# renmengye/rec-attend-public

Hardware: AMD Instinct MI355X
Metric: instance-timesteps/sec, full_model forward 512x512 T=16 (whole job; pipelined throughput: 8 batches in flight per GPU, fill and drain of the pipeline inside the timed region; config.lone_batch_* = one sync-bracketed forward) (higher is better)
Workload: dtype f32; 1 GPU; cfg2: CVPPP-arch full_model eval forward, 512x512, T=16, B=8 per GPU, y_out+s_out; arch=cvppp, H=512, W=512, T=16, batch_per_gpu=8, global_batch=8, parallelism=batch-sharded x1, no collective, ranks_in_communicator=1, hip_graph=True, tile_tickets=False, batches_in_flight=8, pipeline_slots=4, batches_per_launch=2, input=resident in HBM, output=left in HBM

## Files before the change

rec-attend-public_amd/csrc/ra_conv_pair8.hip:

```cpp
#include "ra_conv_pair_parts.h"
#include "ra_split3.h"

namespace ra {
namespace cpair {

template <int CINA>
struct NGeo {
  static constexpr int TH = 16, TW = 32;
  static constexpr int NCGA = CINA / 4;
  static constexpr int AGX = 5, AGY = 5, NGA = AGX * AGY, GPW = (NGA + 3) / 4;
  static constexpr int AW = 41, AHS = TH + 2;
  static constexpr int LW = 43, LH = 4 * AGY + 2;
  static constexpr int LHL = TH + 4, LWL = TW + 6;
  static constexpr int PLANE_B = AHS * AW * 16;
  template <bool CACHED>
  static constexpr int tin_floats() {
    return (LH * LW * (CACHED ? 1 : CINA) + 3) & ~3;
  }
  template <bool SPLIT>
  static constexpr int tmid_floats() {
    return SPLIT ? 3 * PLANE_B / 4 : AHS * AW * 8;
  }
  template <bool CACHED, bool SPLIT>
  static constexpr int lds_floats() {
    return tin_floats<CACHED>() + tmid_floats<SPLIT>();
  }
};

#ifndef RA_PAIR8_OCC
#define RA_PAIR8_OCC 3
#endif
#ifdef RA_PROBE8
__device__ long long *ra_probe8_buf;
#define RA_PHASE_PROBE_BUF ra_probe8_buf
#define RA_PHASE_PROBE_WG blockIdx.x
#endif
#include "ra_phase_probe.h"
#ifdef RA_P8_NOBAR
#define RA_P8_SYNC() __builtin_amdgcn_s_waitcnt(0xc07f)
#else
#define RA_P8_SYNC() __syncthreads()
#endif
template <int CINA, bool CACHED, bool SPLIT = false>
__global__ __launch_bounds__(256, CACHED ? (SPLIT ? 3 : 4) : RA_PAIR8_OCC) void conv_pair8_mfma(const PArgs a, int tiles_x, int tiles_y, int ntiles) {
  using G = NGeo<CINA>;
  constexpr int NCGA = G::NCGA;
  static_assert(!CACHED || CINA == 4, "cached form: 4 input channels");
  static_assert(!SPLIT || CACHED, "the split-precision layer B exists for the cached (steady-state) form");
  constexpr int PLANE_B = G::PLANE_B;
  constexpr int RECA = CACHED ? 1 : CINA;
  extern __shared__ __attribute__((aligned(16))) float lds[];
  constexpr int IN_FLOATS = G::template tin_floats<CACHED>();
  float *tin = lds;
  float *tmid = lds + IN_FLOATS;
  typedef typename vec_of<NCGA>::type avecA;

  const int tid = threadIdx.x, lane = tid & 63;
  __shared__ unsigned tk_sh[2];
  TicketWalk tk;
  const bool dyn = a.tickets != nullptr;
  if (dyn) tk.issue(a.tickets, ntiles);
  const int wave = __builtin_amdgcn_readfirstlane(tid >> 6);
  const int m = lane & 15, ksub = lane >> 4;
  const int n = lane & 15, qo = lane >> 4;
  const int p = n >> 3, co = n & 7;
  const int per = tiles_x * tiles_y;

  const float scA = a.scA[co], scB = a.scB[co], shB = a.shB[co];
  const float loA = a.reluA ? 0.f : -__builtin_inff(), loB = a.reluB ? 0.f : -__builtin_inff();
  const int qA = m >> 2, rA = m & 3, pA = ksub >> 1, coA0 = 4 * (ksub & 1);
  f32x4 scA4, shA4;
#pragma unroll
  for (int j = 0; j < 4; ++j) scA4[j] = a.scA[coA0 + j], shA4[j] = a.shA[coA0 + j];
  const bool fill = !CACHED && a.cache != nullptr;
  float bA[CACHED ? 1 : 12][NCGA], bB[12][2];
  float bAc[3];
#pragma unroll
  for (int ky = 0; ky < 3; ++ky) {
    const int kx = ksub - p;
    const bool ok = (kx >= 0) & (kx <= 2);
    const int tap = ok ? ky * 3 + kx : 0;
    const float w = a.wpA[((tap * NCGA + (a.plane_chan >> 2)) * 4 + (a.plane_chan & 3)) * a.CoutAP + co];
    bAc[ky] = (CACHED && ok) ? w * scA : 0.f;
  }
#pragma unroll
  for (int ky = 0; ky < 3; ++ky)
#pragma unroll
    for (int kxp = 0; kxp < 4; ++kxp) {
      const int kx = kxp - p;
      const bool ok = (kx >= 0) & (kx <= 2);
      const int tap = ok ? ky * 3 + kx : 0;
      if constexpr (!CACHED) {
#pragma unroll
        for (int cg = 0; cg < NCGA; ++cg) {
          const float w = a.wpA[((tap * NCGA + cg) * 4 + ksub) * a.CoutAP + co];
          bA[ky * 4 + kxp][cg] = ok ? w * (fill ? 1.f : scA) : 0.f;
        }
      }
#pragma unroll
      for (int cg = 0; cg < 2; ++cg) {
        const float w = a.wpB[((tap * 2 + cg) * 4 + ksub) * a.CoutBP + co];
        bB[ky * 4 + kxp][cg] = ok ? w * scB : 0.f;
      }
    }

  s16x8 wB[SPLIT ? 3 : 1][SPLIT ? 3 : 1];
  if constexpr (SPLIT) {
#pragma unroll
    for (int ky = 0; ky < 3; ++ky) {
      const int kx = ksub - p;
      const bool ok = (kx >= 0) & (kx <= 2);
      const int tap = ok ? ky * 3 + kx : 0;
#pragma unroll
      for (int j = 0; j < 8; j += 2) {
        const float w0 = a.wpB[((tap * 2 + (j >> 2)) * 4 + (j & 3)) * a.CoutBP + co];
        const float w1 = a.wpB[((tap * 2 + ((j + 1) >> 2)) * 4 + ((j + 1) & 3)) * a.CoutBP + co];
        unsigned H, M, L;
        split3_pair(ok ? w0 * scB : 0.f, ok ? w1 * scB : 0.f, H, M, L);
        wB[ky][0][j] = (short)(H & 0xffffu), wB[ky][0][j + 1] = (short)(H >> 16);
        wB[ky][1][j] = (short)(M & 0xffffu), wB[ky][1][j + 1] = (short)(M >> 16);
        wB[ky][2][j] = (short)(L & 0xffffu), wB[ky][2][j + 1] = (short)(L >> 16);
      }
    }
  }
  const __amdgpu_buffer_rsrc_t rs = __builtin_amdgcn_make_buffer_rsrc(const_cast<float *>(a.src), 0, a.bytes0, 0x00020000);
  const __amdgpu_buffer_rsrc_t rp = __builtin_amdgcn_make_buffer_rsrc(
      const_cast<float *>(a.plane ? a.plane : a.src), 0, a.plane ? a.bytes_p : 0, 0x00020000);
  constexpr int NE = G::LHL * G::LWL, NIT = (NE + 255) / 256;
  int e_rr[NIT], e_cc[NIT];
#pragma unroll
  for (int i = 0; i < NIT; ++i) {
    const int e = tid + 256 * i;
    e_rr[i] = e / G::LWL;
    e_cc[i] = e - e_rr[i] * G::LWL;
    if (e >= NE) e_rr[i] = -(1 << 20);
  }
  unsigned e_offp[NIT], e_offs[NIT];
#pragma unroll
  for (int i = 0; i < NIT; ++i) {
    const bool in = tid + 256 * i < NE;
    const unsigned o = (unsigned)(e_rr[i] * a.W + e_cc[i]) * 4u;
    e_offp[i] = in ? o : 0x80000000u;
    e_offs[i] = in ? o * CINA : 0x80000000u;
  }
  struct TC {
    int b, ty, tx;
  };
  auto split = [&](int t) {
    TC c;
    c.b = t / per;
    const int r = t - c.b * per;
    c.ty = r / tiles_x;
    c.tx = r - c.ty * tiles_x;
    return c;
  };
  const int nwx = a.xcd_map ? (int)gridDim.x >> 3 : (int)gridDim.x;
  const int chunk = (ntiles + 7) >> 3;
  const int t_first = a.xcd_map ? ((int)blockIdx.x & 7) * chunk + ((int)blockIdx.x >> 3) : (int)blockIdx.x;
  const int t_end = a.xcd_map ? (((int)blockIdx.x & 7) * chunk + chunk < ntiles ? ((int)blockIdx.x & 7) * chunk + chunk : ntiles) : ntiles;
  const TC stride = split(nwx);
  auto advance = [&](TC c) {
    c.tx += stride.tx;
    if (c.tx >= tiles_x) {
      c.tx -= tiles_x;
      ++c.ty;
    }
    c.ty += stride.ty;
    if (c.ty >= tiles_y) {
      c.ty -= tiles_y;
      ++c.b;
    }
    c.b += stride.b;
    return c;
  };
  f32x4 v[NIT][NCGA];
  float pv[NIT];
  auto fetch = [&](const TC &c) {
    const int fb = c.b, fy0 = c.ty * G::TH - 2, fx0 = c.tx * G::TW - 3;
    const bool inside = (fy0 >= 0) & (fy0 + G::LHL <= a.H) & (fx0 >= 0) & (fx0 + G::LWL <= a.W);
    if (inside) {
      const unsigned base = (unsigned)((fb * a.H + fy0) * a.W + fx0) * 4u;
#pragma unroll
      for (int i = 0; i < NIT; ++i) {
        if constexpr (!CACHED) {
#pragma unroll
          for (int cg = 0; cg < NCGA; ++cg)
            v[i][cg] = __builtin_bit_cast(
                f32x4, __builtin_amdgcn_raw_buffer_load_b128(rs, (int)(base * CINA + e_offs[i] + 16u * cg), 0, 0));
        }
        pv[i] = __builtin_bit_cast(float, __builtin_amdgcn_raw_buffer_load_b32(rp, (int)(base + e_offp[i]), 0, 0));
      }
      return;
    }
#pragma unroll
    for (int i = 0; i < NIT; ++i) {
      const int Y = fy0 + e_rr[i], X = fx0 + e_cc[i];
      const bool ok = (Y >= 0) & (Y < a.H) & (X >= 0) & (X < a.W);
      const int pix = (fb * a.H + Y) * a.W + X;
      if constexpr (!CACHED) {
#pragma unroll
        for (int cg = 0; cg < NCGA; ++cg)
          v[i][cg] = __builtin_bit_cast(
              f32x4, __builtin_amdgcn_raw_buffer_load_b128(rs, ok ? (pix * CINA + 4 * cg) * 4 : 0x7fffffff, 0, 0));
      }
      pv[i] = __builtin_bit_cast(float, __builtin_amdgcn_raw_buffer_load_b32(rp, ok ? pix * 4 : 0x7fffffff, 0, 0));
    }
  };

  const int lane_in = CACHED ? (m >> 2) * G::LW + 2 * (m & 3) + ksub
                             : ((m >> 2) * G::LW + 2 * (m & 3)) * CINA + ksub * NCGA;
  const __amdgpu_buffer_rsrc_t rc = __builtin_amdgcn_make_buffer_rsrc(
      const_cast<float *>(a.cache ? a.cache : a.src), 0, a.cache ? a.bytes_c : 0, 0x00020000);
  const int lane_b = ((m & 1) * G::AW + 2 * (m >> 1) + 1) * 8 + ksub * 2;
  const int pg = a.plane_chan >> 2, slot = a.plane_chan & 3;

  int slot_c[G::GPW];
#pragma unroll
  for (int s = 0; s < G::GPW; ++s) {
    int gi = wave + 4 * s;
    if (gi >= G::NGA) gi = G::NGA - 1;
    const int gr = gi / G::AGX, gc = gi - gr * G::AGX;
    slot_c[s] = (4 * gr * a.cache_gx + gc) * 256;
  }
  const int lane_c = qA * a.cache_gx * 256 + rA * 64 + ksub * 16;
  const __amdgpu_buffer_rsrc_t ry = __builtin_amdgcn_make_buffer_rsrc(a.y, 0, a.bytes_y, 0x00020000);
  const unsigned lane_y = co < a.CoutB ? (unsigned)(((2 * qo + p) * a.CoutB + co) * 4) : 0x80000000u;
  int g_y[4];
#pragma unroll
  for (int g = 0; g < 4; ++g) g_y[g] = ((g >> 1) * a.Wo + 8 * (g & 1)) * a.CoutB * 4;

  int tile = t_first;
  if (dyn) {
    tk.begin(tk_sh);
    tile = tk.cur;
  }
  bool have = dyn ? tile >= 0 : tile < t_end;
  TC cur = split(have ? tile : 0), nxt = cur;
  if (have) fetch(cur);
  RA_PHASE_DECL;
  for (int e = tid; e < G::template lds_floats<CACHED, SPLIT>() / 4; e += 256)
    reinterpret_cast<f32x4 *>(lds)[e] = f32x4{0.f, 0.f, 0.f, 0.f};
  __syncthreads();
  const bool rider = !CACHED && a.rider_dst != nullptr;
  const __amdgpu_buffer_rsrc_t rr = __builtin_amdgcn_make_buffer_rsrc(rider ? a.rider_dst : a.y, 0,
                                                                       rider ? a.rider_quads * 16 : 0, 0x00020000);
  const int r_chunk = rider ? (a.rider_quads + (int)gridDim.x - 1) / (int)gridDim.x : 0;
  int r_idx = (int)blockIdx.x * r_chunk + tid;
  const int r_end = ((int)blockIdx.x + 1) * r_chunk < a.rider_quads ? ((int)blockIdx.x + 1) * r_chunk : a.rider_quads;
  const int my_tiles = t_end > t_first ? (t_end - t_first + nwx - 1) / nwx : 1;
  const int r_per_tile = (r_chunk + 256 * my_tiles - 1) / (256 * my_tiles);
  const u32x4 r_bits = __builtin_bit_cast(u32x4, f32x4{a.rider_val, a.rider_val, a.rider_val, a.rider_val});
  bool have_n = false;
  f32x4 cpre[CACHED ? G::GPW : 1];
  auto load_cache = [&](const TC &tc) {
    const int tile_c0 = ((tc.b * a.cache_rows + tc.ty * G::TH) * a.cache_gx + ((tc.tx * G::TW) >> 3)) * 256;
#pragma unroll
    for (int s = 0; s < (CACHED ? G::GPW : 1); ++s)
      cpre[s] = __builtin_bit_cast(f32x4, __builtin_amdgcn_raw_buffer_load_b128(rc, tile_c0 + slot_c[s] + lane_c, 0, 0));
  };
  for (; have; tile = dyn ? (tk.step(), tk.cur) : tile + nwx, cur = nxt, have = have_n) {
    const int b = cur.b, ty0 = cur.ty * G::TH, tx0 = cur.tx * G::TW;
    if constexpr (CACHED) load_cache(cur);

#pragma unroll
    for (int i = 0; i < NIT; ++i) {
      if constexpr (CACHED) {
        if (e_rr[i] >= 0) tin[e_rr[i] * G::LW + e_cc[i]] = pv[i];
        continue;
      }
      if (a.plane) {
#pragma unroll
        for (int cg = 0; cg < NCGA; ++cg) {
          v[i][cg].x = (cg == pg && slot == 0) ? pv[i] : v[i][cg].x;
          v[i][cg].y = (cg == pg && slot == 1) ? pv[i] : v[i][cg].y;
          v[i][cg].z = (cg == pg && slot == 2) ? pv[i] : v[i][cg].z;
          v[i][cg].w = (cg == pg && slot == 3) ? pv[i] : v[i][cg].w;
        }
      }
      if (e_rr[i] >= 0) {
        float *rec = tin + (e_rr[i] * G::LW + e_cc[i]) * CINA;
        if constexpr (NCGA == 1) {
          *reinterpret_cast<f32x4 *>(rec) = v[i][0];
        } else {
#pragma unroll
          for (int ks = 0; ks < 4; ++ks)
#pragma unroll
            for (int cg = 0; cg < NCGA; ++cg) rec[ks * NCGA + cg] = v[i][cg][ks];
        }
      }
    }
    if (dyn) tk.publish(tk_sh);
    RA_P8_SYNC();
    RA_PHASE_AT(0);
    if (dyn) {
      tk.read_next(tk_sh);
      tk.request();
      have_n = tk.nxt >= 0;
      nxt = split(have_n ? tk.nxt : 0);
    } else {
      have_n = tile + nwx < t_end;
      nxt = advance(cur);
    }
    if (have_n) fetch(nxt);
    if constexpr (!CACHED) {
      if (rider)
        for (int u = 0; u < r_per_tile; ++u, r_idx += 256)
          __builtin_amdgcn_raw_buffer_store_b128(r_bits, rr, r_idx < r_end ? r_idx * 16 : 0x7fffffff, 0, 0);
    }

    {
      const bool interior = (ty0 >= 1) & (ty0 + G::TH + 1 <= a.H) & (tx0 >= 2) & (tx0 + G::TW + 1 <= a.W);
      const int tile_c = ((b * a.cache_rows + ty0) * a.cache_gx + (tx0 >> 3)) * 256;
      f32x4 acc[G::GPW];
      int gin[G::GPW];
#pragma unroll
      for (int s = 0; s < G::GPW; ++s) {
        int gi = wave + 4 * s;
        if (gi >= G::NGA) gi = G::NGA - 1;
        const int gr = gi / G::AGX, gc = gi - gr * G::AGX;
        gin[s] = (4 * gr * G::LW + 8 * gc) * RECA + lane_in;
        if constexpr (CACHED) {
          acc[s] = cpre[s] * scA4 + shA4;
        } else {
          acc[s] = fill ? f32x4{0.f, 0.f, 0.f, 0.f} : shA4;
        }
      }
      RA_PHASE_AT(1);
      if constexpr (CACHED) {
#pragma unroll
        for (int ky = 0; ky < 3; ++ky) {
          float av[G::GPW];
#pragma unroll
          for (int s = 0; s < G::GPW; ++s) av[s] = tin[gin[s] + ky * G::LW];
#pragma unroll
          for (int s = 0; s < G::GPW; ++s)
            acc[s] = __builtin_amdgcn_mfma_f32_16x16x4f32(bAc[ky], av[s], acc[s], 0, 0, 0);
        }
      } else {
#pragma unroll
      for (int ky = 0; ky < 3; ++ky)
#pragma unroll
        for (int kxp = 0; kxp < 4; ++kxp) {
          avecA av[G::GPW];
#pragma unroll
          for (int s = 0; s < G::GPW; ++s)
            av[s] = *reinterpret_cast<const avecA *>(&tin[gin[s] + (ky * G::LW + kxp) * CINA]);
#pragma unroll
          for (int cg = 0; cg < NCGA; ++cg)
#pragma unroll
            for (int s = 0; s < G::GPW; ++s)
              acc[s] = __builtin_amdgcn_mfma_f32_16x16x4f32(bA[ky * 4 + kxp][cg], av[s][cg], acc[s], 0, 0, 0);
        }
      }
      if (fill) {
#pragma unroll
        for (int s = 0; s < G::GPW; ++s) {
          int gi = wave + 4 * s;
          if (gi >= G::NGA) gi = G::NGA - 1;
          const int gr = gi / G::AGX, gc = gi - gr * G::AGX;
          const bool mine = (4 * gr + qA < G::AHS) & ((gc < 4) | (tx0 + G::TW >= a.W));
          const int off = mine ? tile_c + slot_c[s] + lane_c : 0x7fffffff;
          __builtin_amdgcn_raw_buffer_store_b128(__builtin_bit_cast(__attribute__((ext_vector_type(4))) unsigned, acc[s]), rc, off, 0, 0);
          acc[s] = acc[s] * scA4 + shA4;
        }
      }
#pragma unroll
      for (int s = 0; s < G::GPW; ++s) {
        const int gi = wave + 4 * s;
        const int gr = gi / G::AGX, gc = gi - gr * G::AGX;
        const bool live = (gi < G::NGA) & (4 * gr + qA < G::AHS);
        float o[4];
#pragma unroll
        for (int j = 0; j < 4; ++j) o[j] = fmaxf(acc[s][j], loA);
        if (!interior) {
          const int Y = ty0 - 1 + 4 * gr + qA, X = tx0 - 2 + 8 * gc + 2 * rA + pA;
          const bool ok = (Y >= 0) & (Y < a.H) & (X >= 0) & (X < a.W);
#pragma unroll
          for (int j = 0; j < 4; ++j) o[j] = ok ? o[j] : 0.f;
        }
        const int pix = (4 * gr + qA) * G::AW + 8 * gc + 2 * rA + pA;
        if constexpr (SPLIT) {
          unsigned H01, M01, L01, H23, M23, L23;
          split3_pair(o[0], o[1], H01, M01, L01);
          split3_pair(o[2], o[3], H23, M23, L23);
          if (live) {
            unsigned char *d0 = reinterpret_cast<unsigned char *>(tmid) + pix * 16 + coA0 * 2;
            *reinterpret_cast<u32x2 *>(d0) = u32x2{H01, H23};
            *reinterpret_cast<u32x2 *>(d0 + PLANE_B) = u32x2{M01, M23};
            *reinterpret_cast<u32x2 *>(d0 + 2 * PLANE_B) = u32x2{L01, L23};
          }
        } else if (live) {
          float *dst = tmid + pix * 8 + (ksub & 1);
#pragma unroll
          for (int j = 0; j < 4; ++j) dst[2 * j] = o[j];
        }
      }
    }
    RA_PHASE_AT(2);
    RA_P8_SYNC();
    RA_PHASE_AT(3);

    {
      f32x4 acc[4];
      int gmid[4];
#pragma unroll
      for (int g = 0; g < 4; ++g) {
        const int gy = 2 * wave + (g >> 1), gx = g & 1;
        gmid[g] = (2 * gy * G::AW + 16 * gx) * 8 + lane_b;
        acc[g] = f32x4{shB, shB, shB, shB};
      }
      if constexpr (SPLIT) {
        const unsigned char *tb = reinterpret_cast<const unsigned char *>(tmid);
        const int lane_px = ((m & 1) * G::AW + 2 * (m >> 1) + 1 + ksub) * 16;
#pragma unroll
        for (int ky = 0; ky < 3; ++ky)
#pragma unroll
          for (int gh = 0; gh < 2; ++gh) {
            s16x8 av[2][3];
#pragma unroll
            for (int u = 0; u < 2; ++u) {
              const int g = 2 * gh + u;
              const int gy = 2 * wave + (g >> 1), gx = g & 1;
              const int off = ((2 * gy + ky) * G::AW + 16 * gx) * 16 + lane_px;
#pragma unroll
              for (int pc = 0; pc < 3; ++pc) av[u][pc] = *reinterpret_cast<const s16x8 *>(tb + off + pc * PLANE_B);
            }
            constexpr int PA[6] = {1, 0, 2, 0, 1, 0}, PB[6] = {1, 2, 0, 1, 0, 0};
#pragma unroll
            for (int t = 0; t < 6; ++t)
#pragma unroll
              for (int u = 0; u < 2; ++u)
                acc[2 * gh + u] = __builtin_amdgcn_mfma_f32_16x16x32_bf16(__builtin_bit_cast(bf16x8, av[u][PA[t]]),
                                                                          __builtin_bit_cast(bf16x8, wB[ky][PB[t]]), acc[2 * gh + u], 0, 0, 0);
          }
      } else {
#pragma unroll
      for (int ky = 0; ky < 3; ++ky)
#pragma unroll
        for (int kxp = 0; kxp < 4; ++kxp) {
          f32x2 av[4];
#pragma unroll
          for (int g = 0; g < 4; ++g)
            av[g] = *reinterpret_cast<const f32x2 *>(&tmid[gmid[g] + (ky * G::AW + kxp) * 8]);
#pragma unroll
          for (int cg = 0; cg < 2; ++cg)
#pragma unroll
            for (int g = 0; g < 4; ++g)
              acc[g] = __builtin_amdgcn_mfma_f32_16x16x4f32(av[g][cg], bB[ky * 4 + kxp][cg], acc[g], 0, 0, 0);
        }
      }
      const int prow0 = (ty0 >> 1) + wave * 2, pcol0 = (tx0 >> 1) + 2 * qo + p;
      const bool whole = ((ty0 >> 1) + G::TH / 2 <= a.Ho) & ((tx0 >> 1) + G::TW / 2 <= a.Wo);
      const unsigned tile_y = (unsigned)(((b * a.Ho + prow0) * a.Wo + (tx0 >> 1)) * a.CoutB * 4) + lane_y;
#pragma unroll
      for (int g = 0; g < 4; ++g) {
        const float t0 = fmaxf(fmaxf(acc[g][0], acc[g][1]), loB), t1 = fmaxf(fmaxf(acc[g][2], acc[g][3]), loB);
        const float u0 = fmaxf(t0, __builtin_bit_cast(float, __builtin_amdgcn_mov_dpp(__builtin_bit_cast(int, t0), 0x128, 0xf, 0xf, true)));
        const float u1 = fmaxf(t1, __builtin_bit_cast(float, __builtin_amdgcn_mov_dpp(__builtin_bit_cast(int, t1), 0x128, 0xf, 0xf, true)));
        const float ov = p ? u1 : u0;
        const int prow = prow0 + (g >> 1), pcol = pcol0 + 8 * (g & 1);
        unsigned off = tile_y + (unsigned)g_y[g];
        if (!whole) off = ((prow < a.Ho) & (pcol < a.Wo)) ? off : 0x80000000u;
        __builtin_amdgcn_raw_buffer_store_b32(__builtin_bit_cast(unsigned, ov), ry, (int)off, 0, 0);
      }
    }
    RA_PHASE_AT(4);
  }
  RA_PHASE_END;
  if constexpr (!CACHED) {
    if (rider)
      for (; r_idx < r_end; r_idx += 256) __builtin_amdgcn_raw_buffer_store_b128(r_bits, rr, r_idx * 16, 0, 0);
  }
}

template <int CINA, bool CACHED = false, bool SPLIT = false>
int launch8(PArgs a, int B, hipStream_t st, int *plan) {
  using G = NGeo<CINA>;
  a.bytes_y = (int)((size_t)B * a.Ho * a.Wo * a.CoutB * sizeof(float));
  auto kern = conv_pair8_mfma<CINA, CACHED, SPLIT>;
  constexpr size_t lds = (size_t)G::template lds_floats<CACHED, SPLIT>() * sizeof(float);
  const int tiles_x = ceil_div(a.W, G::TW), tiles_y = ceil_div(a.H, G::TH);
  const int ntiles = tiles_x * tiles_y * B;
  static const int wgs = env_int("RA_PAIR8_WGS", 768);
  static const int xcd = env_int("RA_PAIR8_XCD", 1);
  const int grid = ntiles < wgs ? ntiles : wgs;
  a.xcd_map = (xcd && grid % 8 == 0 && grid >= 8) ? 1 : 0;
  const bool draws = CACHED && ntiles >= kTicketMinTilesPerWg * grid;
  if (plan) {
    plan[RA_PLAN_FAMILY] = RA_PLAN_FAMILY_PAIR;
    plan[RA_PLAN_FORM] = RA_PLAN_FORM_NPACKED | (CACHED ? RA_PLAN_FORM_CACHED : 0) | (SPLIT ? RA_PLAN_FORM_SPLIT : 0);
    plan[RA_PLAN_CK] = CINA, plan[RA_PLAN_CMID] = 8, plan[RA_PLAN_KF] = 3, plan[RA_PLAN_TILE_H] = G::TH, plan[RA_PLAN_TILE_W] = G::TW;
    plan[RA_PLAN_TILES_X] = tiles_x, plan[RA_PLAN_TILES_Y] = tiles_y, plan[RA_PLAN_TICKETS] = draws ? 1 : 0;
    plan_walk(plan, ntiles, grid, a.xcd_map);
    return 0;
  }
  static const MaxDynamicLds lds_limit(kern, lds);
  a.tickets = draws ? take_ticket_slots(1, grid) : nullptr;
  hipLaunchKernelGGL(kern, dim3(grid), dim3(256), lds, st, a, tiles_x, tiles_y, ntiles);
  return launch_status("ra_conv_pair_f32");
}

__global__ __launch_bounds__(256) void first_cache_kernel(const float *x, const float *wpA, int CoutAP, int plane_chan,
                                                          int B, int H, int W, int rows, int ngx, float *cache) {
  __shared__ float sm[4][64][9];
  const int xl = threadIdx.x & 63, yl = threadIdx.x >> 6;
  const int X = blockIdx.x * 64 - 2 + xl, Y = blockIdx.y * 4 + yl, b = blockIdx.z;
  float acc[8];
#pragma unroll
  for (int co = 0; co < 8; ++co) acc[co] = 0.f;
  if (X >= 0 && X < W && Y < H) {
#pragma unroll
    for (int ky = 0; ky < 3; ++ky) {
      const int yy = Y + ky - 1;
#pragma unroll
      for (int kx = 0; kx < 3; ++kx) {
        const int xx = X + kx - 1;
        const bool ok = (yy >= 0) & (yy < H) & (xx >= 0) & (xx < W);
        f32x4 v = f32x4{0.f, 0.f, 0.f, 0.f};
        if (ok) v = *reinterpret_cast<const f32x4 *>(x + ((size_t)(b * H + yy) * W + xx) * 4);
        const float *wt = wpA + (size_t)((ky * 3 + kx) * 4) * CoutAP;
#pragma unroll
        for (int ci = 0; ci < 4; ++ci) {
          const float xv = ci == plane_chan ? 0.f : v[ci];
#pragma unroll
          for (int co = 0; co < 8; ++co) acc[co] = fmaf(xv, wt[ci * CoutAP + co], acc[co]);
        }
      }
    }
  }
#pragma unroll
  for (int co = 0; co < 8; ++co) sm[yl][xl][co] = acc[co];
  __syncthreads();
  for (int e = threadIdx.x; e < 4 * 8 * 16; e += 256) {
    const int n4 = e & 3, r = (e >> 2) & 3, g = (e >> 4) & 7, row = e >> 7;
    const int p = n4 >> 1, co0 = 4 * (n4 & 1);
    const int Yo = blockIdx.y * 4 + row, gx = blockIdx.x * 8 + g;
    if (Yo < H && gx < ngx) {
      f32x4 o;
#pragma unroll
      for (int j = 0; j < 4; ++j) o[j] = sm[row][8 * g + 2 * r + p][co0 + j];
      *reinterpret_cast<f32x4 *>(cache + (((size_t)b * rows + (Yo + 1)) * ngx + gx) * 64 + r * 16 + 4 * n4) = o;
    }
  }
}

void cache_dims(int H, int W, int &rows, int &ngx) {
  rows = ceil_div(H, NGeo<4>::TH) * NGeo<4>::TH + 4;
  ngx = ceil_div(W, NGeo<4>::TW) * (NGeo<4>::TW / 8) + 1;
}
int launch_npacked(const PArgs &a, int B, hipStream_t st, int *plan) {
  return a.C0 == 4 ? launch8<4>(a, B, st, plan) : launch8<8>(a, B, st, plan);
}

int fill_cache_entry(const float *src, const float *plane, int plane_chan, int B, int H, int W, const float *wpA, const float *scaleA,
                     const float *shiftA, int reluA, const float *wpB, const float *scaleB, const float *shiftB, int CoutB, int reluB,
                     float *cache, float *y, float *fill_dst, size_t fill_floats, float fill_value, void *stream, int *plan) {
  if (missing_pointer(plan, {src, plane, cache, wpA, scaleA, shiftA, wpB, scaleB, shiftB, y}) || B <= 0)
    return fail(RA_E_INVALID, "ra_conv_pair_fill_cache_f32: bad argument");
  if (fill_dst && ((reinterpret_cast<uintptr_t>(fill_dst) & 15) || (fill_floats & 3) || fill_floats * 4 >= (1ull << 31)))
    return fail(RA_E_SHAPE, "ra_conv_pair_fill_cache_rider_f32: the fill must be 16-byte aligned, a multiple of 4 floats, < 2 GiB");
  if (!ra_conv_first_cache_supported(4, 8, CoutB, 2, H, W) || plane_chan < 0 || plane_chan > 3)
    return fail(RA_E_SHAPE, "ra_conv_pair_fill_cache_f32: unsupported shape");
  PArgs a = pair_args(src, 4, B, H, W, 0, wpA, scaleA, shiftA, 8, reluA, wpB, scaleB, shiftB, CoutB, reluB, 2, plane, plane_chan, y);
  const size_t b0 = (size_t)B * H * W * 4 * sizeof(float);
  if (b0 >= (1ull << 31)) return fail(RA_E_SHAPE, "ra_conv_pair_fill_cache_f32: input exceeds 2 GiB");
  a.bytes0 = (int)b0;
  if (int rc = pair_args_cache(a, cache, B, "ra_conv_pair_fill_cache_f32")) return rc;
  a.rider_dst = fill_floats ? fill_dst : nullptr;
  a.rider_quads = (int)(fill_floats / 4);
  a.rider_val = fill_value;
  return launch8<4, false>(a, B, as_stream(stream), plan);
}

int cached_entry(const float *cache, const float *plane, int plane_chan, int B, int H, int W, const float *wpA, const float *scaleA,
                 const float *shiftA, int reluA, const float *wpB, const float *scaleB, const float *shiftB, int CoutB, int reluB,
                 float *y, void *stream, int *plan) {
  if (missing_pointer(plan, {cache, plane, wpA, scaleA, shiftA, wpB, scaleB, shiftB, y}) || B <= 0)
    return fail(RA_E_INVALID, "ra_conv_pair_cached_f32: bad argument");
  if (!ra_conv_first_cache_supported(4, 8, CoutB, 2, H, W) || plane_chan < 0 || plane_chan > 3)
    return fail(RA_E_SHAPE, "ra_conv_pair_cached_f32: unsupported shape");
  PArgs a = pair_args(plane, 4, B, H, W, 0, wpA, scaleA, shiftA, 8, reluA, wpB, scaleB, shiftB, CoutB, reluB, 2, plane, plane_chan, y);
  if (int rc = pair_args_cache(a, cache, B, "ra_conv_pair_cached_f32")) return rc;
  static const int split = env_int("RA_PAIR8_SPLIT", 1);
  if (split) return launch8<4, true, true>(a, B, as_stream(stream), plan);
  return launch8<4, true>(a, B, as_stream(stream), plan);
}

}
}

using namespace ra;

extern "C" int ra_conv_first_cache_supported(int Cin, int CoutA, int CoutB, int poolB, int H, int W) {
  return Cin == 4 && CoutA == 8 && CoutB >= 1 && CoutB <= 8 && poolB == 2 && W > 16 && !((H | W) & 1);
}

extern "C" size_t ra_conv_first_cache_floats(int B, int H, int W) {
  if (B <= 0 || H <= 0 || W <= 0) return 0;
  int rows, ngx;
  cpair::cache_dims(H, W, rows, ngx);
  return (size_t)B * rows * ngx * 64;
}

extern "C" int ra_conv_first_cache_f32(const float *src, int B, int H, int W, const float *wpA, int CoutA,
                                       int plane_chan, float *cache, void *stream) {
  if (!src || !wpA || !cache || B <= 0 || H <= 0 || W <= 0 || plane_chan < 0 || plane_chan > 3)
    return fail(RA_E_INVALID, "ra_conv_first_cache_f32: bad argument");
  if (CoutA != 8) return fail(RA_E_SHAPE, "ra_conv_first_cache_f32: CoutA %d", CoutA);
  int rows, ngx;
  cpair::cache_dims(H, W, rows, ngx);
  const size_t total = (size_t)B * rows * ngx * 16;
  if (total * 16 >= (1ull << 31)) return fail(RA_E_SHAPE, "ra_conv_first_cache_f32: cache exceeds 2 GiB");
  hipLaunchKernelGGL(cpair::first_cache_kernel, dim3(ceil_div(W + 2, 64), ceil_div(H, 4), B), dim3(256), 0,
                     as_stream(stream), src, wpA, ra_conv_cout_padded(CoutA), plane_chan, B, H, W, rows, ngx, cache);
  return launch_status("ra_conv_first_cache_f32");
}

extern "C" int ra_conv_pair_fill_cache_rider_f32(const float *src, const float *plane, int plane_chan, int B, int H, int W,
                                                 const float *wpA, const float *scaleA, const float *shiftA, int reluA,
                                                 const float *wpB, const float *scaleB, const float *shiftB, int CoutB,
                                                 int reluB, float *cache, float *y, float *fill_dst, size_t fill_floats,
                                                 float fill_value, void *stream) {
  return cpair::fill_cache_entry(src, plane, plane_chan, B, H, W, wpA, scaleA, shiftA, reluA, wpB, scaleB, shiftB, CoutB, reluB, cache, y,
                                 fill_dst, fill_floats, fill_value, stream, nullptr);
}

extern "C" int ra_conv_pair_fill_cache_f32(const float *src, const float *plane, int plane_chan, int B, int H, int W,
                                           const float *wpA, const float *scaleA, const float *shiftA, int reluA,
                                           const float *wpB, const float *scaleB, const float *shiftB, int CoutB,
                                           int reluB, float *cache, float *y, void *stream) {
  return ra_conv_pair_fill_cache_rider_f32(src, plane, plane_chan, B, H, W, wpA, scaleA, shiftA, reluA, wpB, scaleB, shiftB,
                                           CoutB, reluB, cache, y, nullptr, 0, 0.0f, stream);
}

extern "C" int ra_conv_pair_cached_f32(const float *cache, const float *plane, int plane_chan, int B, int H, int W,
                                       const float *wpA, const float *scaleA, const float *shiftA, int reluA,
                                       const float *wpB, const float *scaleB, const float *shiftB, int CoutB,
                                       int reluB, float *y, void *stream) {
  return cpair::cached_entry(cache, plane, plane_chan, B, H, W, wpA, scaleA, shiftA, reluA, wpB, scaleB, shiftB, CoutB, reluB, y, stream,
                             nullptr);
}
```

Before: 57490 instance-timesteps/s.

## Remap phase-A MFMA groups to cover 18x18 pair-rows with 21 groups

Replaces the 5x5 grid of phase-A MFMA groups (25 groups, 7 per wave, many lanes dead on the 18-row/20-pair overhang) with an exact mapping of 21 groups over the 18x18 pair-row area. Each wave now runs 5 groups, and one corner group is rotated across waves per tile. A constexpr check verifies the coverage is exact. The aim is fewer wasted MFMAs, LDS reads and cache loads/stores in phase A, at the cost of more complex per-lane address math and some wave imbalance on the corner group.

Measured after the change: 59600 instance-timesteps/s (median of 6 runs). 1.04x the previous value.

```diff
diff --git a/rec-attend-public_amd/csrc/ra_conv_pair8.hip b/rec-attend-public_amd/csrc/ra_conv_pair8.hip
--- a/rec-attend-public_amd/csrc/ra_conv_pair8.hip
+++ b/rec-attend-public_amd/csrc/ra_conv_pair8.hip
@@ -1,3 +1,5 @@
+#include <type_traits>
+
 #include "ra_conv_pair_parts.h"
 #include "ra_split3.h"
 
@@ -8,10 +10,42 @@
 struct NGeo {
   static constexpr int TH = 16, TW = 32;
   static constexpr int NCGA = CINA / 4;
-  static constexpr int AGX = 5, AGY = 5, NGA = AGX * AGY, GPW = (NGA + 3) / 4;
   static constexpr int AW = 41, AHS = TH + 2;
-  static constexpr int LW = 43, LH = 4 * AGY + 2;
+  static constexpr int LW = 43, LH = 22;
+  static constexpr int NGA = 21, GPW = 5, NSLOT = GPW + 1, AR = AHS, AP = TW / 2 + 2;
+  struct Cell {
+    int row, pair;
+    bool live;
+  };
+  static constexpr __host__ __device__ int group_of(int wave, int s) { return s < 4 ? 4 * s + wave : s == 4 ? 16 + wave : 20; }
+  static constexpr __host__ __device__ Cell cell(int wave, int s, int m) {
+    if (s < 4) return Cell{4 * s + (m >> 2), 4 * wave + (m & 3), true};
+    if (s == 4) return wave < 2 ? Cell{8 * wave + (m >> 1), 16 + (m & 1), true} : Cell{16 + (m >> 3), 8 * (wave - 2) + (m & 7), true};
+    return Cell{16 + ((m >> 1) & 1), 16 + (m & 1), m < 4};
+  }
+  static constexpr bool map_exact() {
+    int hits[AR * AP] = {};
+    bool seen[NGA] = {};
+    for (int s = 0; s < NSLOT; ++s)
+      for (int w = 0; w < (s == GPW ? 1 : 4); ++w) {
+        const int g = group_of(w, s);
+        if (g < 0 || g >= NGA || seen[g]) return false;
+        seen[g] = true;
+        for (int m = 0; m < 16; ++m) {
+          const Cell c = cell(w, s, m);
+          if (c.row < 0 || c.row >= AR || c.pair < 0 || c.pair >= AP) return false;
+          if (c.live) ++hits[c.row * AP + c.pair];
+        }
+      }
+    for (int g = 0; g < NGA; ++g)
+      if (!seen[g]) return false;
+    for (int i = 0; i < AR * AP; ++i)
+      if (hits[i] != 1) return false;
+    return true;
+  }
+  static_assert(AR * AP == 324 && NGA * 16 - 12 == AR * AP, "18 rows x 18 pairs = 21 groups less the corner's 12 spare rows");
   static constexpr int LHL = TH + 4, LWL = TW + 6;
+  static_assert(AR - 1 + 2 < LHL && 2 * (AP - 1) + 3 < LWL && LHL <= LH && LWL <= LW, "every cell's 3 x 4 window is staged");
   static constexpr int PLANE_B = AHS * AW * 16;
   template <bool CACHED>
   static constexpr int tin_floats() {
@@ -26,6 +60,7 @@
     return tin_floats<CACHED>() + tmid_floats<SPLIT>();
   }
 };
+static_assert(NGeo<4>::map_exact() && NGeo<8>::map_exact(), "phase A's groups cover the 18 x 18 pair-rows exactly once");
 
 #ifndef RA_PAIR8_OCC
 #define RA_PAIR8_OCC 3
@@ -68,7 +103,7 @@
 
   const float scA = a.scA[co], scB = a.scB[co], shB = a.shB[co];
   const float loA = a.reluA ? 0.f : -__builtin_inff(), loB = a.reluB ? 0.f : -__builtin_inff();
-  const int qA = m >> 2, rA = m & 3, pA = ksub >> 1, coA0 = 4 * (ksub & 1);
+  const int pA = ksub >> 1, coA0 = 4 * (ksub & 1);
   f32x4 scA4, shA4;
 #pragma unroll
   for (int j = 0; j < 4; ++j) scA4[j] = a.scA[coA0 + j], shA4[j] = a.shA[coA0 + j];
@@ -207,22 +242,32 @@
     }
   };
 
-  const int lane_in = CACHED ? (m >> 2) * G::LW + 2 * (m & 3) + ksub
-                             : ((m >> 2) * G::LW + 2 * (m & 3)) * CINA + ksub * NCGA;
   const __amdgpu_buffer_rsrc_t rc = __builtin_amdgcn_make_buffer_rsrc(
       const_cast<float *>(a.cache ? a.cache : a.src), 0, a.cache ? a.bytes_c : 0, 0x00020000);
   const int lane_b = ((m & 1) * G::AW + 2 * (m >> 1) + 1) * 8 + ksub * 2;
   const int pg = a.plane_chan >> 2, slot = a.plane_chan & 3;
 
-  int slot_c[G::GPW];
-#pragma unroll
-  for (int s = 0; s < G::GPW; ++s) {
-    int gi = wave + 4 * s;
-    if (gi >= G::NGA) gi = G::NGA - 1;
-    const int gr = gi / G::AGX, gc = gi - gr * G::AGX;
-    slot_c[s] = (4 * gr * a.cache_gx + gc) * 256;
-  }
-  const int lane_c = qA * a.cache_gx * 256 + rA * 64 + ksub * 16;
+  struct LaneCell {
+    int in, c, pix;
+  };
+  auto lane_cell = [&](int s, int mm) {
+    const typename G::Cell c = G::cell(wave, s, mm);
+    return LaneCell{(c.row * G::LW + 2 * c.pair) * RECA + ksub * (CACHED ? 1 : NCGA),
+                    (c.row * a.cache_gx + (c.pair >> 2)) * 256 + (c.pair & 3) * 64 + ksub * 16, c.row * G::AW + 2 * c.pair + pA};
+  };
+  auto lane_rowcol = [&](int s) {
+    int mm = m;
+    asm volatile("" : "+v"(mm));
+    const typename G::Cell c = G::cell(wave, s, mm);
+    return c.row | (2 * c.pair + pA) << 8;
+  };
+  const LaneCell cell_i = lane_cell(0, m), cell_s = lane_cell(G::GPW - 1, m);
+  auto corner_cell = [&]() {
+    int mm = m;
+    asm volatile("" : "+v"(mm));
+    return lane_cell(G::GPW, mm);
+  };
+  const int rows4_c = 4 * a.cache_gx * 256;
   const __amdgpu_buffer_rsrc_t ry = __builtin_amdgcn_make_buffer_rsrc(a.y, 0, a.bytes_y, 0x00020000);
   const unsigned lane_y = co < a.CoutB ? (unsigned)(((2 * qo + p) * a.CoutB + co) * 4) : 0x80000000u;
   int g_y[4];
@@ -251,16 +296,24 @@
   const int r_per_tile = (r_chunk + 256 * my_tiles - 1) / (256 * my_tiles);
   const u32x4 r_bits = __builtin_bit_cast(u32x4, f32x4{a.rider_val, a.rider_val, a.rider_val, a.rider_val});
   bool have_n = false;
-  f32x4 cpre[CACHED ? G::GPW : 1];
-  auto load_cache = [&](const TC &tc) {
+  f32x4 cpre[CACHED ? G::NSLOT : 1];
+  LaneCell cell_c{};
+  auto load_cache = [&](const TC &tc, bool own) {
     const int tile_c0 = ((tc.b * a.cache_rows + tc.ty * G::TH) * a.cache_gx + ((tc.tx * G::TW) >> 3)) * 256;
 #pragma unroll
     for (int s = 0; s < (CACHED ? G::GPW : 1); ++s)
-      cpre[s] = __builtin_bit_cast(f32x4, __builtin_amdgcn_raw_buffer_load_b128(rc, tile_c0 + slot_c[s] + lane_c, 0, 0));
+      cpre[s] = __builtin_bit_cast(f32x4, __builtin_amdgcn_raw_buffer_load_b128(
+                                              rc, tile_c0 + (s < 4 ? s * rows4_c + cell_i.c : cell_s.c), 0, 0));
+    if constexpr (CACHED)
+      if (own) {
+        cell_c = corner_cell();
+        cpre[G::GPW] = __builtin_bit_cast(f32x4, __builtin_amdgcn_raw_buffer_load_b128(rc, tile_c0 + cell_c.c, 0, 0));
+      }
   };
   for (; have; tile = dyn ? (tk.step(), tk.cur) : tile + nwx, cur = nxt, have = have_n) {
     const int b = cur.b, ty0 = cur.ty * G::TH, tx0 = cur.tx * G::TW;
-    if constexpr (CACHED) load_cache(cur);
+    const bool own = wave == (tile & 3);
+    if constexpr (CACHED) load_cache(cur, own);
 
 #pragma unroll
     for (int i = 0; i < NIT; ++i) {
@@ -311,89 +364,90 @@
     {
       const bool interior = (ty0 >= 1) & (ty0 + G::TH + 1 <= a.H) & (tx0 >= 2) & (tx0 + G::TW + 1 <= a.W);
       const int tile_c = ((b * a.cache_rows + ty0) * a.cache_gx + (tx0 >> 3)) * 256;
-      f32x4 acc[G::GPW];
-      int gin[G::GPW];
-#pragma unroll
-      for (int s = 0; s < G::GPW; ++s) {
-        int gi = wave + 4 * s;
-        if (gi >= G::NGA) gi = G::NGA - 1;
-        const int gr = gi / G::AGX, gc = gi - gr * G::AGX;
-        gin[s] = (4 * gr * G::LW + 8 * gc) * RECA + lane_in;
+      auto groups = [&](auto s0c, auto s1c, const LaneCell &edge, int rowcol_i, int rowcol_e) __attribute__((always_inline)) {
+        constexpr int S0 = decltype(s0c)::value, NS = decltype(s1c)::value - S0;
+        f32x4 acc[NS];
+        int gin[NS];
+#pragma unroll
+        for (int s = 0; s < NS; ++s) gin[s] = S0 + s < 4 ? cell_i.in + 4 * (S0 + s) * G::LW * RECA : edge.in;
+#pragma unroll
+        for (int s = 0; s < NS; ++s) {
+          if constexpr (CACHED) {
+            acc[s] = cpre[S0 + s] * scA4 + shA4;
+          } else {
+            acc[s] = fill ? f32x4{0.f, 0.f, 0.f, 0.f} : shA4;
+          }
+        }
+        if constexpr (S0 == 0) RA_PHASE_AT(1);
         if constexpr (CACHED) {
-          acc[s] = cpre[s] * scA4 + shA4;
+#pragma unroll
+          for (int ky = 0; ky < 3; ++ky) {
+            float av[NS];
+#pragma unroll
+            for (int s = 0; s < NS; ++s) av[s] = tin[gin[s] + ky * G::LW];
+#pragma unroll
+            for (int s = 0; s < NS; ++s)
+              acc[s] = __builtin_amdgcn_mfma_f32_16x16x4f32(bAc[ky], av[s], acc[s], 0, 0, 0);
+          }
         } else {
-          acc[s] = fill ? f32x4{0.f, 0.f, 0.f, 0.f} : shA4;
-        }
-      }
-      RA_PHASE_AT(1);
-      if constexpr (CACHED) {
-#pragma unroll
-        for (int ky = 0; ky < 3; ++ky) {
-          float av[G::GPW];
-#pragma unroll
-          for (int s = 0; s < G::GPW; ++s) av[s] = tin[gin[s] + ky * G::LW];
-#pragma unroll
-          for (int s = 0; s < G::GPW; ++s)
-            acc[s] = __builtin_amdgcn_mfma_f32_16x16x4f32(bAc[ky], av[s], acc[s], 0, 0, 0);
-        }
-      } else {
-#pragma unroll
-      for (int ky = 0; ky < 3; ++ky)
-#pragma unroll
-        for (int kxp = 0; kxp < 4; ++kxp) {
-          avecA av[G::GPW];
-#pragma unroll
-          for (int s = 0; s < G::GPW; ++s)
-            av[s] = *reinterpret_cast<const avecA *>(&tin[gin[s] + (ky * G::LW + kxp) * CINA]);
-#pragma unroll
-          for (int cg = 0; cg < NCGA; ++cg)
-#pragma unroll
-            for (int s = 0; s < G::GPW; ++s)
-              acc[s] = __builtin_amdgcn_mfma_f32_16x16x4f32(bA[ky * 4 + kxp][cg], av[s][cg], acc[s], 0, 0, 0);
-        }
-      }
-      if (fill) {
-#pragma unroll
-        for (int s = 0; s < G::GPW; ++s) {
-          int gi = wave + 4 * s;
-          if (gi >= G::NGA) gi = G::NGA - 1;
-          const int gr = gi / G::AGX, gc = gi - gr * G::AGX;
-          const bool mine = (4 * gr + qA < G::AHS) & ((gc < 4) | (tx0 + G::TW >= a.W));
-          const int off = mine ? tile_c + slot_c[s] + lane_c : 0x7fffffff;
-          __builtin_amdgcn_raw_buffer_store_b128(__builtin_bit_cast(__attribute__((ext_vector_type(4))) unsigned, acc[s]), rc, off, 0, 0);
-          acc[s] = acc[s] * scA4 + shA4;
-        }
-      }
-#pragma unroll
-      for (int s = 0; s < G::GPW; ++s) {
-        const int gi = wave + 4 * s;
-        const int gr = gi / G::AGX, gc = gi - gr * G::AGX;
-        const bool live = (gi < G::NGA) & (4 * gr + qA < G::AHS);
-        float o[4];
-#pragma unroll
-        for (int j = 0; j < 4; ++j) o[j] = fmaxf(acc[s][j], loA);
-        if (!interior) {
-          const int Y = ty0 - 1 + 4 * gr + qA, X = tx0 - 2 + 8 * gc + 2 * rA + pA;
-          const bool ok = (Y >= 0) & (Y < a.H) & (X >= 0) & (X < a.W);
-#pragma unroll
-          for (int j = 0; j < 4; ++j) o[j] = ok ? o[j] : 0.f;
-        }
-        const int pix = (4 * gr + qA) * G::AW + 8 * gc + 2 * rA + pA;
-        if constexpr (SPLIT) {
-          unsigned H01, M01, L01, H23, M23, L23;
-          split3_pair(o[0], o[1], H01, M01, L01);
-          split3_pair(o[2], o[3], H23, M23, L23);
-          if (live) {
-            unsigned char *d0 = reinterpret_cast<unsigned char *>(tmid) + pix * 16 + coA0 * 2;
-            *reinterpret_cast<u32x2 *>(d0) = u32x2{H01, H23};
-            *reinterpret_cast<u32x2 *>(d0 + PLANE_B) = u32x2{M01, M23};
-            *reinterpret_cast<u32x2 *>(d0 + 2 * PLANE_B) = u32x2{L01, L23};
+#pragma unroll
+          for (int ky = 0; ky < 3; ++ky)
+#pragma unroll
+            for (int kxp = 0; kxp < 4; ++kxp) {
+              avecA av[NS];
+#pragma unroll
+              for (int s = 0; s < NS; ++s)
+                av[s] = *reinterpret_cast<const avecA *>(&tin[gin[s] + (ky * G::LW + kxp) * CINA]);
+#pragma unroll
+              for (int cg = 0; cg < NCGA; ++cg)
+#pragma unroll
+                for (int s = 0; s < NS; ++s)
+                  acc[s] = __builtin_amdgcn_mfma_f32_16x16x4f32(bA[ky * 4 + kxp][cg], av[s][cg], acc[s], 0, 0, 0);
+            }
+        }
+#pragma unroll
+        for (int s = 0; s < NS; ++s) {
+          const int S = S0 + s < 4 ? S0 + s : 0;
+          const bool inner = S0 + s < 4;
+          const bool live = S0 + s < G::GPW || m < 4;
+          if (fill) {
+            const int off = live ? tile_c + (inner ? S * rows4_c + cell_i.c : edge.c) : 0x7fffffff;
+            __builtin_amdgcn_raw_buffer_store_b128(__builtin_bit_cast(__attribute__((ext_vector_type(4))) unsigned, acc[s]), rc, off, 0, 0);
+            acc[s] = acc[s] * scA4 + shA4;
           }
-        } else if (live) {
-          float *dst = tmid + pix * 8 + (ksub & 1);
-#pragma unroll
-          for (int j = 0; j < 4; ++j) dst[2 * j] = o[j];
-        }
+          float o[4];
+#pragma unroll
+          for (int j = 0; j < 4; ++j) o[j] = fmaxf(acc[s][j], loA);
+          if (!interior) {
+            const int rowcol = inner ? rowcol_i + 4 * S : rowcol_e;
+            const int Y = ty0 - 1 + (rowcol & 255), X = tx0 - 2 + (rowcol >> 8);
+            const bool ok = (Y >= 0) & (Y < a.H) & (X >= 0) & (X < a.W);
+#pragma unroll
+            for (int j = 0; j < 4; ++j) o[j] = ok ? o[j] : 0.f;
+          }
+          const int pix = inner ? cell_i.pix + 4 * S * G::AW : edge.pix;
+          if constexpr (SPLIT) {
+            unsigned H01, M01, L01, H23, M23, L23;
+            split3_pair(o[0], o[1], H01, M01, L01);
+            split3_pair(o[2], o[3], H23, M23, L23);
+            if (live) {
+              unsigned char *d0 = reinterpret_cast<unsigned char *>(tmid) + pix * 16 + coA0 * 2;
+              *reinterpret_cast<u32x2 *>(d0) = u32x2{H01, H23};
+              *reinterpret_cast<u32x2 *>(d0 + PLANE_B) = u32x2{M01, M23};
+              *reinterpret_cast<u32x2 *>(d0 + 2 * PLANE_B) = u32x2{L01, L23};
+            }
+          } else if (live) {
+            float *dst = tmid + pix * 8 + (ksub & 1);
+#pragma unroll
+            for (int j = 0; j < 4; ++j) dst[2 * j] = o[j];
+          }
+        }
+      };
+      groups(std::integral_constant<int, 0>{}, std::integral_constant<int, G::GPW>{}, cell_s, interior ? 0 : lane_rowcol(0),
+             interior ? 0 : lane_rowcol(G::GPW - 1));
+      if (own) {
+        if constexpr (!CACHED) cell_c = corner_cell();
+        groups(std::integral_constant<int, G::GPW>{}, std::integral_constant<int, G::NSLOT>{}, cell_c, 0, interior ? 0 : lane_rowcol(G::GPW));
       }
     }
     RA_PHASE_AT(2);
```
